# anacarsi/ss25_Hierarchical_Multiscale_Image_Classification

Measured on AMD Instinct MI355X. Metric: 224x224 patches/sec (ResNet18 fwd), higher is better.
Workload: dtype bf16; 1 GPU; resnet18_fwd_872k_patches_bf16; input=uint8 HWC patches resident in HBM, outputs=features[B,512] + logits[B,2] + labels, weights=seeded random init, parallelism=single GPU

## Files before the change

ss25_hierarchical_multiscale_image_classification_amd/csrc/block16_c64.h:

```cpp
#pragma once
#include "halo16.h"

namespace hipac {

typedef __attribute__((ext_vector_type(2))) short s16x2;
__device__ __forceinline__ unsigned relu_pk(unsigned v) {
  return __builtin_bit_cast(unsigned, __builtin_elementwise_max(__builtin_bit_cast(s16x2, v), s16x2{0, 0}));
}

constexpr int kBlkRing = 30;
constexpr int kBlkXPitch = 18 * 128;
constexpr int kBlkIPitch = 16 * 128;
constexpr int kBlkXBytes = 32 * kBlkXPitch + 512;
constexpr int kBlkIBytes = 32 * kBlkIPitch + 256;
constexpr int kBlkRsBytes = 2 * 6144 + 2 * 4096;

#ifndef HIPAC_BLK16_AHEAD
#define HIPAC_BLK16_AHEAD 1
#endif

template <typename T, int NP, int PITCH>
__device__ __forceinline__ void c64_strip16_mfma(const typename Elem<T>::frag (&wreg)[9][2][2], const int (&lb)[NP][3],
                                                 const float* __restrict__ bl, f32x4 (&acc)[2 * NP][2]) {
  using frag = typename Elem<T>::frag;
  constexpr int NR = 2 * NP;
#pragma unroll
  for (int t = 0; t < 2; ++t) {
    const f32x4 b = *reinterpret_cast<const f32x4*>(bl + 16 * t);
#pragma unroll
    for (int i = 0; i < NR; ++i) acc[i][t] = b;
  }
  asm volatile("s_waitcnt lgkmcnt(0)" ::: "memory");
  constexpr int AH = HIPAC_BLK16_AHEAD;
  frag fr[AH + 1][NR];
  auto rd = [&](auto S, auto I) {
    constexpr int s = decltype(S)::value, i = decltype(I)::value;
    constexpr int tap = s >> 1, kk = s & 1, kh = tap / 3, kw = tap % 3;
    lds_read16<((i & 1) + kh) * PITCH>(fr[s % (AH + 1)][i], (unsigned)(lb[i >> 1][kw] ^ (kk << 6)));
  };
  __builtin_amdgcn_s_setprio(1);
  static_for<AH>([&](auto S) { static_for<NR>([&](auto I) { rd(S, I); }); });
  static_for<18>([&](auto S) {
    constexpr int s = decltype(S)::value, tap = s >> 1, kk = s & 1;
    static_for<NR>([&](auto I) {
      constexpr int i = decltype(I)::value;
      if constexpr (s + AH < 18) rd(std::integral_constant<int, s + AH>{}, I);
      constexpr int full = (18 - 1 - s < AH - 1 ? 18 - 1 - s : AH - 1);
      wait_lgkmcnt<(NR - 1 - i) + full * NR + (s + AH < 18 ? i + 1 : 0)>();
      Asm16<T>::mfma(acc[i][0], wreg[tap][kk][0], fr[s % (AH + 1)][i]);
      Asm16<T>::mfma(acc[i][1], wreg[tap][kk][1], fr[s % (AH + 1)][i]);
    });
  });
  __builtin_amdgcn_s_setprio(0);
  asm volatile("s_nop 7\n\ts_nop 7\n\ts_nop 3" ::: "memory");
}

template <typename T>
__global__ __launch_bounds__(512, 2) void block16_c64_kernel(const T* __restrict__ in, const T* __restrict__ w1,
                                                             const float* __restrict__ b1, const T* __restrict__ w2,
                                                             const float* __restrict__ b2, T* __restrict__ out,
                                                             int n_img) {
  using E = Elem<T>;
  using frag = typename E::frag;
  using vec4 = typename E::vec4;
  constexpr int H = 56, W = 56, C = 64, RING = kBlkRing, XP = kBlkXPitch, IP = kBlkIPitch;
  __shared__ __attribute__((aligned(1024))) unsigned char smem[kBlkXBytes + kBlkIBytes + kBlkRsBytes + 512];
  unsigned char* const Xr = smem;
  unsigned char* const Ir = smem + kBlkXBytes;
  float* const Bl = reinterpret_cast<float*>(smem + kBlkXBytes + kBlkIBytes + kBlkRsBytes);

  const int tid = threadIdx.x, lane = tid & 63;
  const int wave = __builtin_amdgcn_readfirstlane(tid >> 6);
  const int team = wave >> 2, tw = wave & 3, nh = tw & 1, mh = tw >> 1;
  const int n16 = lane & 15, g = lane >> 4;
  const int lx = n16 < 4 ? 2 * n16 : (n16 < 12 ? 2 * n16 - 7 : 2 * n16 - 16);
  unsigned char* const Rw = smem + kBlkXBytes + kBlkIBytes + (mh == 0 ? nh * 6144 : 2 * 6144 + nh * 4096);

  if (tid < 64) Bl[tid] = b1[tid];
  else if (tid < 128) Bl[tid] = b2[tid - 64];

  const int xcd = blockIdx.x & 7, slot = blockIdx.x >> 3, nslots = gridDim.x >> 3;
  const int n_x = n_img > xcd ? (n_img - xcd + 7) >> 3 : 0;
  const int nst = 4 * n_x;
  const int ns = nst > slot ? (nst - slot + nslots - 1) / nslots : 0;
  if (ns == 0) return;

  frag wreg[9][2][2];
  {
    const char* wb = reinterpret_cast<const char*>(team ? w2 : w1) + (size_t)(nh * 32 + n16) * (9 * C * 2) + 16 * g;
#pragma unroll
    for (int tap = 0; tap < 9; ++tap)
#pragma unroll
      for (int kk = 0; kk < 2; ++kk)
#pragma unroll
        for (int t = 0; t < 2; ++t) wreg[tap][kk][t] = *reinterpret_cast<const frag*>(wb + t * 16 * (9 * C * 2) + tap * 128 + kk * 64);
  }

  const rsrc_t x_rsrc = make_rsrc(in, n_img * (H * W * C * 2));

  constexpr int NKP = 5;
  int relo[NKP];
#pragma unroll
  for (int kp = 0; kp < NKP; ++kp) {
    const int q = 8 * (tw + 4 * kp) + (lane >> 3);
    const int rr = (q * 3641) >> 16;
    const int j = q - 18 * rr;
    const int c = (lane & 7) ^ ((j >> 1) & 7);
    relo[kp] = (((rr * W + j) << 7) + (c << 4)) | (j < 2 ? 1 : 0) | (j >= 16 ? 2 : 0) | (rr == 0 ? 4 : 0) | (rr >= 1 ? 8 : 0);
  }
  auto x_rows = [&](int img, int x0, int L0, int rb, int np, int rowmask) {
    const int sb = ((img * H + L0 - 1) * W + x0 - 2) << 7;
    const int smask = (x0 == 0 ? 1 : 0) | (x0 == 42 ? 2 : 0) | rowmask;
    static_for<NKP>([&](auto KP) {
      constexpr int kp = decltype(KP)::value;
      const int p = tw + 4 * kp;
      if (p < np) {
        asm volatile("" : "+v"(relo[kp]));
        const int off = (relo[kp] & smask) ? (int)0x80000000 : (relo[kp] & ~15) + sb;
        buffer_load_lds16(x_rsrc, Xr + rb * XP + p * 1024, off, 0);
      }
    });
  };
  auto x_group = [&](int img, int x0, int gq) {
    const int rb = 8 * gq >= RING ? 8 * gq - RING : 8 * gq;
    x_rows(img, x0, 8 * gq, rb, gq == 7 ? 5 : 18, gq == 0 ? 4 : (gq == 7 ? 8 : 0));
    if (gq == 3) x_rows(img, x0, RING, 0, 5, 0);
  };
  auto strip_img = [&](int k) { return (((slot + k * nslots) >> 2) << 3) + xcd; };
  auto strip_x0 = [&](int k) { return ((slot + k * nslots) & 3) * 14; };

  const int lds_base = (int)(unsigned)(size_t)(__attribute__((address_space(3))) unsigned char*)smem;
  int la[3];
#pragma unroll
  for (int kw = 0; kw < 3; ++kw) {
    const int j = lx + kw;
    la[kw] = (j << 7) + (((((j >> 1) & 7)) ^ g) << 4) + (team ? kBlkXBytes : 0) + lds_base;
  }
  const int iw_lane = (lx << 7) + ((g & 1) << 3);
  const int iw_pos = ((nh << 2) + (g >> 1)) ^ ((lx >> 1) & 7);
  const float* const bl = Bl + team * 64 + nh * 32 + 4 * g;

#pragma unroll
  for (int tap = 0; tap < 9; ++tap)
#pragma unroll
    for (int kk = 0; kk < 2; ++kk)
#pragma unroll
      for (int t = 0; t < 2; ++t) asm volatile("" ::"v"(wreg[tap][kk][t]));
  if (team == 0) {
    x_group(strip_img(0), strip_x0(0), 0);
    x_group(strip_img(0), strip_x0(0), 1);
    wait_vmcnt<0>();
  }
  asm volatile("s_waitcnt lgkmcnt(0)" ::: "memory");
  __builtin_amdgcn_s_barrier();

  const int n_steps = 7 * ns;
  f32x4 acc[4][2];
  int pend_n = 0, pend_y = 0;
  const int rs_px = lane >> 2;
  const int rs_off = (((rs_px < 14 ? rs_px : 13)) * C + nh * 32 + 8 * ((lane & 3) ^ ((rs_px >> 2) & 3))) * 2;
  auto fetch_resid = [&](int pix0, int y0, int sl) {
    const int sb = (pix0 + y0 * W) << 7;
#pragma unroll
    for (int rho = 0; rho < 2; ++rho) buffer_load_lds16(x_rsrc, Rw + sl * 2048 + rho * 1024, rs_off + rho * (W * C * 2), sb);
  };
  const int rs_rd = lx * 64 + 8 * (g & 1);
  const int rs_sw = (lx >> 2) & 3;
  const int out_lane = (lx * C + nh * 32 + 16 * (g & 1) + 8 * (g >> 1)) * 2;
  auto epilogue_b = [&](auto A0, int pix0, int y0, int sl) {
    constexpr int a0 = decltype(A0)::value;
#pragma unroll
    for (int rho = 0; rho < 2; ++rho) {
      unsigned P[2][2];
#pragma unroll
      for (int t = 0; t < 2; ++t) {
        const vec4 rv = *reinterpret_cast<const vec4*>(Rw + sl * 2048 + rho * 1024 + rs_rd + (((2 * t + (g >> 1)) ^ rs_sw) << 4));
        const f32x4& a = acc[a0 + rho][t];
        P[t][0] = relu_pk(PackPair<T>::pack_rn(a[0] + (float)rv[0], a[1] + (float)rv[1]));
        P[t][1] = relu_pk(PackPair<T>::pack_rn(a[2] + (float)rv[2], a[3] + (float)rv[3]));
      }
      permlane16_swap(P[0][0], P[1][0]);
      permlane16_swap(P[0][1], P[1][1]);
      char* const dst = reinterpret_cast<char*>(out) + ((size_t)(unsigned)(pix0 + (y0 + rho) * W) << 7) + out_lane;
      if (lx < 14) store16_out(dst, u32x4{P[0][0], P[0][1], P[1][0], P[1][1]});
    }
  };
  int pend_pix = 0, pend_sl = 0;
  auto flush_b = [&]() {
    if (pend_n) {
      wait_vmcnt<0>();
      epilogue_b(std::integral_constant<int, 0>{}, pend_pix, pend_y, pend_sl);
      if (pend_n == 2) epilogue_b(std::integral_constant<int, 2>{}, pend_pix, pend_y + 2, pend_sl + 1);
      pend_n = 0;
    }
  };
  auto step_barrier = [&]() {
    asm volatile("s_waitcnt lgkmcnt(0)" ::: "memory");
    __builtin_amdgcn_s_barrier();
  };
  if (team == 0) {
    for (int G = 0; G <= n_steps; ++G) {
      if (G < n_steps) {
        const int k = G / 7, m = G - 7 * k;
        const int img = strip_img(k), x0 = strip_x0(k);
        if (m <= 4) x_group(img, x0, m + 2);
        else if (m == 5) {
          x_group(img, x0, 7);
          if (k + 1 < ns) x_group(strip_img(k + 1), strip_x0(k + 1), 0);
        } else if (k + 1 < ns) x_group(strip_img(k + 1), strip_x0(k + 1), 1);
        if (m == 0 || m == 6)
          *reinterpret_cast<u32x2*>(Ir + (m == 0 ? 0 : 27) * IP + tw * 512 + lane * 8) = u32x2{0u, 0u};
        const int y0a = 8 * m + 4 * mh;
        int lb[2][3];
#pragma unroll
        for (int p = 0; p < 2; ++p) {
          const int y0 = y0a + 2 * p;
          const int wbase = (y0 >= RING ? y0 - RING : y0) * XP;
#pragma unroll
          for (int kw = 0; kw < 3; ++kw) lb[p][kw] = la[kw] + wbase;
        }
        c64_strip16_mfma<T, 2, XP>(wreg, lb, bl, acc);
        const bool col_ok = !((x0 == 0 && lx == 0) || (x0 == 42 && lx == 15));
#pragma unroll
        for (int i = 0; i < 4; ++i) {
          const int Lr = y0a + i + 1;
          const bool twice = Lr == RING || Lr == RING + 1;
          unsigned char* const dst = Ir + (Lr >= RING ? Lr - RING : Lr) * IP + iw_lane;
          unsigned char* const dst2 = Ir + Lr * IP + iw_lane;
#pragma unroll
          for (int t = 0; t < 2; ++t) {
            u32x2 pk;
            pk[0] = relu_pk(PackPair<T>::pack_rn(acc[i][t][0], acc[i][t][1]));
            pk[1] = relu_pk(PackPair<T>::pack_rn(acc[i][t][2], acc[i][t][3]));
            if (!col_ok) pk = u32x2{0u, 0u};
            *reinterpret_cast<u32x2*>(dst + ((iw_pos ^ (2 * t)) << 4)) = pk;
            if (twice) *reinterpret_cast<u32x2*>(dst2 + ((iw_pos ^ (2 * t)) << 4)) = pk;
          }
        }
      }
      wait_vmcnt<0>();
      step_barrier();
    }
  } else {
    for (int G = 0; G <= n_steps; ++G) {
      flush_b();
      if (G >= 1) {
        const int k = (G - 1) / 7, mp = G - 7 * k;
        int yp = 8 * mp - 10 + 4 * mh, ys = -1;
        bool has_pair = true;
        if (mp == 1) {
          if (mh == 0) yp = 0;
          else has_pair = false, ys = 4;
        } else if (mp == 7) {
          if (mh == 0) yp = 46, ys = 50;
          else yp = 52;
        }
        const int pix0 = strip_img(k) * (H * W) + strip_x0(k);
        if (has_pair) {
          fetch_resid(pix0, yp, 0);
          fetch_resid(pix0, yp + 2, 1);
        }
        if (ys >= 0) fetch_resid(pix0, ys, has_pair ? 2 : 0);
        pend_pix = pix0;
        if (has_pair) {
          int lb[2][3];
#pragma unroll
          for (int p = 0; p < 2; ++p) {
            const int y0 = yp + 2 * p;
            const int wbase = (y0 >= RING ? y0 - RING : y0) * IP;
#pragma unroll
            for (int kw = 0; kw < 3; ++kw) lb[p][kw] = la[kw] + wbase;
          }
          c64_strip16_mfma<T, 2, IP>(wreg, lb, bl, acc);
          pend_n = 2, pend_y = yp, pend_sl = 0;
        }
        if (ys >= 0) {
          flush_b();
          int lb[1][3];
          const int wbase = (ys >= RING ? ys - RING : ys) * IP;
#pragma unroll
          for (int kw = 0; kw < 3; ++kw) lb[0][kw] = la[kw] + wbase;
          f32x4(&acc1)[2][2] = reinterpret_cast<f32x4(&)[2][2]>(acc[0]);
          c64_strip16_mfma<T, 1, IP>(wreg, lb, bl, acc1);
          pend_n = 1, pend_y = ys, pend_sl = has_pair ? 2 : 0;
        }
      }
      step_barrier();
    }
    flush_b();
  }
}

}
```

ss25_hierarchical_multiscale_image_classification_amd/csrc/conv_bf16.hip:

```cpp
#include "trunk.h"
namespace hipac {
int run_trunk_bf16(const Net& net, const Plan& p, char* ws, const void* xin, int n_early, int img_off, int n_late,
                   hipStream_t s, int first, int last) {
  return run_trunk<__bf16>(net, p, ws, xin, n_early, img_off, n_late, s, first, last);
}
}

#ifdef HIPAC_HALO_STAMPS
extern "C" int hipac_debug_halo_stamps(unsigned long long* out8, int reset) {
  if (hipMemcpyFromSymbol(out8, HIP_SYMBOL(hipac::g_halo_stamps), 64) != hipSuccess) return 1;
  if (reset) {
    unsigned long long z[8] = {0};
    if (hipMemcpyToSymbol(HIP_SYMBOL(hipac::g_halo_stamps), z, 64) != hipSuccess) return 1;
  }
  return 0;
}
#endif
```

Measured before the change: 309,200 patches/s.

## Read residual shortcut from X ring in LDS instead of reloading from HBM

The second conv team now takes the residual input from the already-resident X ring buffer in LDS rather than issuing separate buffer loads into a dedicated residual staging area. To keep the needed rows alive long enough, the X ring grows to 32 rows plus 2 wrap rows, indexed per strip with a 58-row stride, and the load scheduling is rewritten around spans. This removes the redundant global reads, the residual LDS region and the vmcnt waits in the epilogue. In exchange it adds more complex ring indexing, a slightly larger X buffer, and extra LDS reads in team B.

Measured after the change: 311,100 patches/s (median of 6 runs). No clear change (+0.6%).

```diff
diff --git a/ss25_hierarchical_multiscale_image_classification_amd/csrc/block16_c64.h b/ss25_hierarchical_multiscale_image_classification_amd/csrc/block16_c64.h
--- a/ss25_hierarchical_multiscale_image_classification_amd/csrc/block16_c64.h
+++ b/ss25_hierarchical_multiscale_image_classification_amd/csrc/block16_c64.h
@@ -1,4 +1,5 @@
 #pragma once
+#include "block16_ring.h"
 #include "halo16.h"
 
 namespace hipac {
@@ -9,11 +10,8 @@
 }
 
 constexpr int kBlkRing = 30;
-constexpr int kBlkXPitch = 18 * 128;
 constexpr int kBlkIPitch = 16 * 128;
-constexpr int kBlkXBytes = 32 * kBlkXPitch + 512;
 constexpr int kBlkIBytes = 32 * kBlkIPitch + 256;
-constexpr int kBlkRsBytes = 2 * 6144 + 2 * 4096;
 
 #ifndef HIPAC_BLK16_AHEAD
 #define HIPAC_BLK16_AHEAD 1
@@ -64,17 +62,16 @@
   using frag = typename E::frag;
   using vec4 = typename E::vec4;
   constexpr int H = 56, W = 56, C = 64, RING = kBlkRing, XP = kBlkXPitch, IP = kBlkIPitch;
-  __shared__ __attribute__((aligned(1024))) unsigned char smem[kBlkXBytes + kBlkIBytes + kBlkRsBytes + 512];
+  __shared__ __attribute__((aligned(1024))) unsigned char smem[kBlkXBytes + kBlkIBytes + 512];
   unsigned char* const Xr = smem;
   unsigned char* const Ir = smem + kBlkXBytes;
-  float* const Bl = reinterpret_cast<float*>(smem + kBlkXBytes + kBlkIBytes + kBlkRsBytes);
+  float* const Bl = reinterpret_cast<float*>(smem + kBlkXBytes + kBlkIBytes);
 
   const int tid = threadIdx.x, lane = tid & 63;
   const int wave = __builtin_amdgcn_readfirstlane(tid >> 6);
   const int team = wave >> 2, tw = wave & 3, nh = tw & 1, mh = tw >> 1;
   const int n16 = lane & 15, g = lane >> 4;
   const int lx = n16 < 4 ? 2 * n16 : (n16 < 12 ? 2 * n16 - 7 : 2 * n16 - 16);
-  unsigned char* const Rw = smem + kBlkXBytes + kBlkIBytes + (mh == 0 ? nh * 6144 : 2 * 6144 + nh * 4096);
 
   if (tid < 64) Bl[tid] = b1[tid];
   else if (tid < 128) Bl[tid] = b2[tid - 64];
@@ -106,28 +103,36 @@
     const int rr = (q * 3641) >> 16;
     const int j = q - 18 * rr;
     const int c = (lane & 7) ^ ((j >> 1) & 7);
-    relo[kp] = (((rr * W + j) << 7) + (c << 4)) | (j < 2 ? 1 : 0) | (j >= 16 ? 2 : 0) | (rr == 0 ? 4 : 0) | (rr >= 1 ? 8 : 0);
-  }
-  auto x_rows = [&](int img, int x0, int L0, int rb, int np, int rowmask) {
+    relo[kp] = (((rr * W + j) << 7) + (c << 4)) | (j < 2 ? 1 : 0) | (j >= 16 ? 2 : 0) | (rr == 0 ? 4 : 0);
+  }
+  auto x_rows = [&](int img, int x0, int L0, int rb, int np) {
     const int sb = ((img * H + L0 - 1) * W + x0 - 2) << 7;
-    const int smask = (x0 == 0 ? 1 : 0) | (x0 == 42 ? 2 : 0) | rowmask;
+    const int smask = (x0 == 0 ? 1 : 0) | (x0 == 42 ? 2 : 0) | (L0 == 0 ? 4 : 0);
+    const int below = (H + 1 - L0) * (W * 128);
     static_for<NKP>([&](auto KP) {
       constexpr int kp = decltype(KP)::value;
       const int p = tw + 4 * kp;
       if (p < np) {
         asm volatile("" : "+v"(relo[kp]));
-        const int off = (relo[kp] & smask) ? (int)0x80000000 : (relo[kp] & ~15) + sb;
+        const int off = ((relo[kp] & smask) || relo[kp] >= below) ? (int)0x80000000 : (relo[kp] & ~15) + sb;
         buffer_load_lds16(x_rsrc, Xr + rb * XP + p * 1024, off, 0);
       }
     });
-  };
-  auto x_group = [&](int img, int x0, int gq) {
-    const int rb = 8 * gq >= RING ? 8 * gq - RING : 8 * gq;
-    x_rows(img, x0, 8 * gq, rb, gq == 7 ? 5 : 18, gq == 0 ? 4 : (gq == 7 ? 8 : 0));
-    if (gq == 3) x_rows(img, x0, RING, 0, 5, 0);
   };
   auto strip_img = [&](int k) { return (((slot + k * nslots) >> 2) << 3) + xcd; };
   auto strip_x0 = [&](int k) { return ((slot + k * nslots) & 3) * 14; };
+  auto x_request = [&](int k, int L0, int nrows) {
+    const int img = strip_img(k), x0 = strip_x0(k);
+#pragma unroll
+    for (int i = 0; i < 3; ++i) {
+      const Blk16Span sp = blk16_x_span(k, L0, nrows, i);
+      if (sp.nrows) x_rows(img, x0, sp.L0, sp.row, blk16_x_pieces(sp.nrows));
+    }
+  };
+  auto x_strip_head = [&](int k) {
+    x_request(k, 0, 2);
+    x_request(k, 2, 8);
+  };
 
   const int lds_base = (int)(unsigned)(size_t)(__attribute__((address_space(3))) unsigned char*)smem;
   int la[3];
@@ -147,8 +152,7 @@
 #pragma unroll
       for (int t = 0; t < 2; ++t) asm volatile("" ::"v"(wreg[tap][kk][t]));
   if (team == 0) {
-    x_group(strip_img(0), strip_x0(0), 0);
-    x_group(strip_img(0), strip_x0(0), 1);
+    x_strip_head(0);
     wait_vmcnt<0>();
   }
   asm volatile("s_waitcnt lgkmcnt(0)" ::: "memory");
@@ -157,27 +161,35 @@
   const int n_steps = 7 * ns;
   f32x4 acc[4][2];
   int pend_n = 0, pend_y = 0;
-  const int rs_px = lane >> 2;
-  const int rs_off = (((rs_px < 14 ? rs_px : 13)) * C + nh * 32 + 8 * ((lane & 3) ^ ((rs_px >> 2) & 3))) * 2;
-  auto fetch_resid = [&](int pix0, int y0, int sl) {
-    const int sb = (pix0 + y0 * W) << 7;
-#pragma unroll
-    for (int rho = 0; rho < 2; ++rho) buffer_load_lds16(x_rsrc, Rw + sl * 2048 + rho * 1024, rs_off + rho * (W * C * 2), sb);
-  };
-  const int rs_rd = lx * 64 + 8 * (g & 1);
-  const int rs_sw = (lx >> 2) & 3;
+  const int sc_j = lx + 2;
+  const int sc_lane = (sc_j << 7) + ((g & 1) << 3);
+  const int sc_pos = ((nh << 2) + (g >> 1)) ^ ((sc_j >> 1) & 7);
   const int out_lane = (lx * C + nh * 32 + 16 * (g & 1) + 8 * (g >> 1)) * 2;
-  auto epilogue_b = [&](auto A0, int pix0, int y0, int sl) {
+  auto add_shortcut = [&](auto NR_, int k, int y0) {
+    constexpr int NR = decltype(NR_)::value;
+    vec4 rv[NR][2];
+#pragma unroll
+    for (int i = 0; i < NR; ++i)
+#pragma unroll
+      for (int t = 0; t < 2; ++t)
+        rv[i][t] = *reinterpret_cast<const vec4*>(Xr + blk16_x_row(k, y0 + i + 1) * XP + sc_lane + ((sc_pos ^ (2 * t)) << 4));
+#pragma unroll
+    for (int i = 0; i < NR; ++i)
+#pragma unroll
+      for (int t = 0; t < 2; ++t)
+#pragma unroll
+        for (int e = 0; e < 4; ++e) acc[i][t][e] = acc[i][t][e] + (float)rv[i][t][e];
+  };
+  auto epilogue_b = [&](auto A0, int pix0, int y0) {
     constexpr int a0 = decltype(A0)::value;
 #pragma unroll
     for (int rho = 0; rho < 2; ++rho) {
       unsigned P[2][2];
 #pragma unroll
       for (int t = 0; t < 2; ++t) {
-        const vec4 rv = *reinterpret_cast<const vec4*>(Rw + sl * 2048 + rho * 1024 + rs_rd + (((2 * t + (g >> 1)) ^ rs_sw) << 4));
         const f32x4& a = acc[a0 + rho][t];
-        P[t][0] = relu_pk(PackPair<T>::pack_rn(a[0] + (float)rv[0], a[1] + (float)rv[1]));
-        P[t][1] = relu_pk(PackPair<T>::pack_rn(a[2] + (float)rv[2], a[3] + (float)rv[3]));
+        P[t][0] = relu_pk(PackPair<T>::pack_rn(a[0], a[1]));
+        P[t][1] = relu_pk(PackPair<T>::pack_rn(a[2], a[3]));
       }
       permlane16_swap(P[0][0], P[1][0]);
       permlane16_swap(P[0][1], P[1][1]);
@@ -185,12 +197,11 @@
       if (lx < 14) store16_out(dst, u32x4{P[0][0], P[0][1], P[1][0], P[1][1]});
     }
   };
-  int pend_pix = 0, pend_sl = 0;
+  int pend_pix = 0;
   auto flush_b = [&]() {
     if (pend_n) {
-      wait_vmcnt<0>();
-      epilogue_b(std::integral_constant<int, 0>{}, pend_pix, pend_y, pend_sl);
-      if (pend_n == 2) epilogue_b(std::integral_constant<int, 2>{}, pend_pix, pend_y + 2, pend_sl + 1);
+      epilogue_b(std::integral_constant<int, 0>{}, pend_pix, pend_y);
+      if (pend_n == 2) epilogue_b(std::integral_constant<int, 2>{}, pend_pix, pend_y + 2);
       pend_n = 0;
     }
   };
@@ -202,20 +213,16 @@
     for (int G = 0; G <= n_steps; ++G) {
       if (G < n_steps) {
         const int k = G / 7, m = G - 7 * k;
-        const int img = strip_img(k), x0 = strip_x0(k);
-        if (m <= 4) x_group(img, x0, m + 2);
-        else if (m == 5) {
-          x_group(img, x0, 7);
-          if (k + 1 < ns) x_group(strip_img(k + 1), strip_x0(k + 1), 0);
-        } else if (k + 1 < ns) x_group(strip_img(k + 1), strip_x0(k + 1), 1);
+        const int x0 = strip_x0(k);
+        if (m <= 5) x_request(k, 8 * m + 10, 8);
+        else if (k + 1 < ns) x_strip_head(k + 1);
         if (m == 0 || m == 6)
           *reinterpret_cast<u32x2*>(Ir + (m == 0 ? 0 : 27) * IP + tw * 512 + lane * 8) = u32x2{0u, 0u};
         const int y0a = 8 * m + 4 * mh;
         int lb[2][3];
 #pragma unroll
         for (int p = 0; p < 2; ++p) {
-          const int y0 = y0a + 2 * p;
-          const int wbase = (y0 >= RING ? y0 - RING : y0) * XP;
+          const int wbase = blk16_x_row(k, y0a + 2 * p) * XP;
 #pragma unroll
           for (int kw = 0; kw < 3; ++kw) lb[p][kw] = la[kw] + wbase;
         }
@@ -246,22 +253,10 @@
       flush_b();
       if (G >= 1) {
         const int k = (G - 1) / 7, mp = G - 7 * k;
-        int yp = 8 * mp - 10 + 4 * mh, ys = -1;
-        bool has_pair = true;
-        if (mp == 1) {
-          if (mh == 0) yp = 0;
-          else has_pair = false, ys = 4;
-        } else if (mp == 7) {
-          if (mh == 0) yp = 46, ys = 50;
-          else yp = 52;
-        }
-        const int pix0 = strip_img(k) * (H * W) + strip_x0(k);
-        if (has_pair) {
-          fetch_resid(pix0, yp, 0);
-          fetch_resid(pix0, yp + 2, 1);
-        }
-        if (ys >= 0) fetch_resid(pix0, ys, has_pair ? 2 : 0);
-        pend_pix = pix0;
+        const Blk16BRows br = blk16_b_rows(mp, mh);
+        const int yp = br.yp, ys = br.ys;
+        const bool has_pair = br.has_pair;
+        pend_pix = strip_img(k) * (H * W) + strip_x0(k);
         if (has_pair) {
           int lb[2][3];
 #pragma unroll
@@ -272,7 +267,8 @@
             for (int kw = 0; kw < 3; ++kw) lb[p][kw] = la[kw] + wbase;
           }
           c64_strip16_mfma<T, 2, IP>(wreg, lb, bl, acc);
-          pend_n = 2, pend_y = yp, pend_sl = 0;
+          add_shortcut(std::integral_constant<int, 4>{}, k, yp);
+          pend_n = 2, pend_y = yp;
         }
         if (ys >= 0) {
           flush_b();
@@ -282,7 +278,8 @@
           for (int kw = 0; kw < 3; ++kw) lb[0][kw] = la[kw] + wbase;
           f32x4(&acc1)[2][2] = reinterpret_cast<f32x4(&)[2][2]>(acc[0]);
           c64_strip16_mfma<T, 1, IP>(wreg, lb, bl, acc1);
-          pend_n = 1, pend_y = ys, pend_sl = has_pair ? 2 : 0;
+          add_shortcut(std::integral_constant<int, 2>{}, k, ys);
+          pend_n = 1, pend_y = ys;
         }
       }
       step_barrier();
diff --git a/ss25_hierarchical_multiscale_image_classification_amd/csrc/block16_ring.h b/ss25_hierarchical_multiscale_image_classification_amd/csrc/block16_ring.h
--- /dev/null
+++ b/ss25_hierarchical_multiscale_image_classification_amd/csrc/block16_ring.h
@@ -0,0 +1,42 @@
+#pragma once
+
+namespace hipac {
+
+constexpr int kBlkXPitch = 18 * 128;
+constexpr int kBlkXRing = 32;
+constexpr int kBlkXRows = kBlkXRing + 2;
+constexpr int kBlkXBytes = kBlkXRows * kBlkXPitch + 512;
+constexpr int kBlkStripRows = 58;
+
+constexpr int blk16_x_row(int strip, int L) { return (kBlkStripRows * strip + L) & (kBlkXRing - 1); }
+constexpr int blk16_x_pieces(int nrows) { return (nrows * 18 + 7) >> 3; }
+
+struct Blk16Span {
+  int L0, row, nrows;
+};
+constexpr Blk16Span blk16_x_span(int strip, int L0, int nrows, int i) {
+  const int r0 = blk16_x_row(strip, L0);
+  const int n1 = nrows < kBlkXRing - r0 ? nrows : kBlkXRing - r0;
+  if (i == 0) return Blk16Span{L0, r0, n1};
+  if (i == 1) return Blk16Span{L0 + n1, 0, nrows - n1};
+  if (r0 == 0) return Blk16Span{L0, kBlkXRing, 2};
+  return Blk16Span{L0 + n1, kBlkXRing, n1 < nrows ? 2 : 0};
+}
+
+struct Blk16BRows {
+  int yp, ys;
+  bool has_pair;
+};
+constexpr Blk16BRows blk16_b_rows(int mp, int mh) {
+  Blk16BRows r{8 * mp - 10 + 4 * mh, -1, true};
+  if (mp == 1) {
+    if (mh == 0) r.yp = 0;
+    else r.has_pair = false, r.ys = 4;
+  } else if (mp == 7) {
+    if (mh == 0) r.yp = 46, r.ys = 50;
+    else r.yp = 52;
+  }
+  return r;
+}
+
+}
```

## Deepen LDS prefetch pipeline in block16 conv MFMA loop and prioritize flush

Applied to the files above, without the earlier changes.

Replaces the per-tap fragment prefetch (one step ahead) with a flat ring of 8 fragment registers and a configurable prefetch distance of 6 reads, so LDS loads run further ahead of the MFMAs. Bias is now loaded with LDS reads into the last accumulator and copied into the others, so its wait folds into the first fragment wait instead of a full lgkmcnt(0) drain. The residual epilogue hoists all LDS residual reads before the math and raises wave priority during the flush. Optional timestamp instrumentation is added behind a debug macro. The deeper ring raises VGPR pressure, which could hurt occupancy under the 512x2 launch bounds.

Result: no change. 311,200 patches/s before, 314,100 patches/s after, median of 6 (+0.9%).

```diff
diff --git a/ss25_hierarchical_multiscale_image_classification_amd/csrc/block16_c64.h b/ss25_hierarchical_multiscale_image_classification_amd/csrc/block16_c64.h
--- a/ss25_hierarchical_multiscale_image_classification_amd/csrc/block16_c64.h
+++ b/ss25_hierarchical_multiscale_image_classification_amd/csrc/block16_c64.h
@@ -14,42 +14,57 @@
 constexpr int kBlkXBytes = 32 * kBlkXPitch + 512;
 constexpr int kBlkIBytes = 32 * kBlkIPitch + 256;
 constexpr int kBlkRsBytes = 2 * 6144 + 2 * 4096;
-
-#ifndef HIPAC_BLK16_AHEAD
-#define HIPAC_BLK16_AHEAD 1
-#endif
-
-template <typename T, int NP, int PITCH>
+constexpr int kBlkStampPairs = 12;
+#ifdef HIPAC_HALO_STAMPS
+static __device__ unsigned long long g_blk16_stamps[20];
+#endif
+
+#ifndef HIPAC_BLK16_DIST
+#define HIPAC_BLK16_DIST 6
+#endif
+#ifndef HIPAC_BLK16_PRIO_FLUSH
+#define HIPAC_BLK16_PRIO_FLUSH 3
+#endif
+
+template <typename T, int NP, int PITCH, typename Mark>
 __device__ __forceinline__ void c64_strip16_mfma(const typename Elem<T>::frag (&wreg)[9][2][2], const int (&lb)[NP][3],
-                                                 const float* __restrict__ bl, f32x4 (&acc)[2 * NP][2]) {
+                                                 unsigned bl, f32x4 (&acc)[2 * NP][2], Mark&& mark) {
   using frag = typename Elem<T>::frag;
   constexpr int NR = 2 * NP;
-#pragma unroll
-  for (int t = 0; t < 2; ++t) {
-    const f32x4 b = *reinterpret_cast<const f32x4*>(bl + 16 * t);
-#pragma unroll
-    for (int i = 0; i < NR; ++i) acc[i][t] = b;
-  }
-  asm volatile("s_waitcnt lgkmcnt(0)" ::: "memory");
-  constexpr int AH = HIPAC_BLK16_AHEAD;
-  frag fr[AH + 1][NR];
-  auto rd = [&](auto S, auto I) {
-    constexpr int s = decltype(S)::value, i = decltype(I)::value;
+  constexpr int NF = 18 * NR;
+  constexpr int R = 8, D = HIPAC_BLK16_DIST;
+  static_assert(D >= 1 && D <= R - 2, "a slot is rewritten two MFMA pairs after its reader at the earliest");
+  static_assert(D + 2 < 16, "lgkmcnt range");
+  frag fr[R];
+  auto rd = [&](auto F) {
+    constexpr int f = decltype(F)::value, s = f / NR, i = f % NR;
     constexpr int tap = s >> 1, kk = s & 1, kh = tap / 3, kw = tap % 3;
-    lds_read16<((i & 1) + kh) * PITCH>(fr[s % (AH + 1)][i], (unsigned)(lb[i >> 1][kw] ^ (kk << 6)));
-  };
+    lds_read16<((i & 1) + kh) * PITCH>(fr[f % R], (unsigned)(lb[i >> 1][kw] ^ (kk << 6)));
+  };
+  asm volatile("" ::: "memory");
   __builtin_amdgcn_s_setprio(1);
-  static_for<AH>([&](auto S) { static_for<NR>([&](auto I) { rd(S, I); }); });
-  static_for<18>([&](auto S) {
-    constexpr int s = decltype(S)::value, tap = s >> 1, kk = s & 1;
-    static_for<NR>([&](auto I) {
-      constexpr int i = decltype(I)::value;
-      if constexpr (s + AH < 18) rd(std::integral_constant<int, s + AH>{}, I);
-      constexpr int full = (18 - 1 - s < AH - 1 ? 18 - 1 - s : AH - 1);
-      wait_lgkmcnt<(NR - 1 - i) + full * NR + (s + AH < 18 ? i + 1 : 0)>();
-      Asm16<T>::mfma(acc[i][0], wreg[tap][kk][0], fr[s % (AH + 1)][i]);
-      Asm16<T>::mfma(acc[i][1], wreg[tap][kk][1], fr[s % (AH + 1)][i]);
-    });
+  lds_read16<0>(acc[NR - 1][0], bl);
+  lds_read16<64>(acc[NR - 1][1], bl);
+  static_for<(D < NF ? D : NF)>([&](auto F) { rd(F); });
+  static_for<NF>([&](auto F) {
+    constexpr int f = decltype(F)::value, s = f / NR, i = f % NR, tap = s >> 1, kk = s & 1;
+    if constexpr (f == kBlkStampPairs) mark(std::integral_constant<int, 1>{});
+    if constexpr (f == NF - kBlkStampPairs) mark(std::integral_constant<int, 2>{});
+    if constexpr (f + D < NF) rd(std::integral_constant<int, f + D>{});
+    constexpr int behind = NF - 1 - f < D ? NF - 1 - f : D;
+    if constexpr (f == 0) {
+      asm volatile("s_waitcnt lgkmcnt(%2)" : "+v"(acc[NR - 1][0]), "+v"(acc[NR - 1][1]) : "n"(behind));
+      mark(std::integral_constant<int, 0>{});
+    } else {
+      wait_lgkmcnt<behind>();
+    }
+    if constexpr (f < NR - 1) {
+      if constexpr (f > 0) asm volatile("" : "+v"(acc[NR - 1][0]), "+v"(acc[NR - 1][1]));
+      acc[i][0] = acc[NR - 1][0];
+      acc[i][1] = acc[NR - 1][1];
+    }
+    Asm16<T>::mfma(acc[i][0], wreg[tap][kk][0], fr[f % R]);
+    Asm16<T>::mfma(acc[i][1], wreg[tap][kk][1], fr[f % R]);
   });
   __builtin_amdgcn_s_setprio(0);
   asm volatile("s_nop 7\n\ts_nop 7\n\ts_nop 3" ::: "memory");
@@ -138,7 +153,7 @@
   }
   const int iw_lane = (lx << 7) + ((g & 1) << 3);
   const int iw_pos = ((nh << 2) + (g >> 1)) ^ ((lx >> 1) & 7);
-  const float* const bl = Bl + team * 64 + nh * 32 + 4 * g;
+  const unsigned bl = (unsigned)(lds_base + kBlkXBytes + kBlkIBytes + kBlkRsBytes + (team * 64 + nh * 32 + 4 * g) * 4);
 
 #pragma unroll
   for (int tap = 0; tap < 9; ++tap)
@@ -155,6 +170,19 @@
   __builtin_amdgcn_s_barrier();
 
   const int n_steps = 7 * ns;
+#ifdef HIPAC_HALO_STAMPS
+  unsigned long long z_sum[11] = {0, 0, 0, 0, 0, 0, 0, 0, 0, 0, 0}, z_tf = 0, z_th = 0, z_tt = 0, z_tv = 0, z_tr = 0;
+  auto mark = [&](auto K) {
+    HALO_STAMP(z_now);
+    if constexpr (decltype(K)::value == 2) z_tt = z_now;
+    else if constexpr (decltype(K)::value == 1) z_th = z_th ? z_th : z_now;
+    else z_tf = z_tf ? z_tf : z_now;
+  };
+  HALO_STAMP(z_t0v);
+  unsigned long long z_t0 = z_t0v;
+#else
+  auto mark = [](auto) {};
+#endif
   f32x4 acc[4][2];
   int pend_n = 0, pend_y = 0;
   const int rs_px = lane >> 2;
@@ -167,14 +195,21 @@
   const int rs_rd = lx * 64 + 8 * (g & 1);
   const int rs_sw = (lx >> 2) & 3;
   const int out_lane = (lx * C + nh * 32 + 16 * (g & 1) + 8 * (g >> 1)) * 2;
-  auto epilogue_b = [&](auto A0, int pix0, int y0, int sl) {
+  auto resid_rows = [&](vec4 (&rv)[2][2], int sl) {
+#pragma unroll
+    for (int rho = 0; rho < 2; ++rho)
+#pragma unroll
+      for (int t = 0; t < 2; ++t)
+        rv[rho][t] = *reinterpret_cast<const vec4*>(Rw + sl * 2048 + rho * 1024 + rs_rd + (((2 * t + (g >> 1)) ^ rs_sw) << 4));
+  };
+  auto epilogue_b = [&](auto A0, int pix0, int y0, const vec4 (&rvs)[2][2]) {
     constexpr int a0 = decltype(A0)::value;
 #pragma unroll
     for (int rho = 0; rho < 2; ++rho) {
       unsigned P[2][2];
 #pragma unroll
       for (int t = 0; t < 2; ++t) {
-        const vec4 rv = *reinterpret_cast<const vec4*>(Rw + sl * 2048 + rho * 1024 + rs_rd + (((2 * t + (g >> 1)) ^ rs_sw) << 4));
+        const vec4 rv = rvs[rho][t];
         const f32x4& a = acc[a0 + rho][t];
         P[t][0] = relu_pk(PackPair<T>::pack_rn(a[0] + (float)rv[0], a[1] + (float)rv[1]));
         P[t][1] = relu_pk(PackPair<T>::pack_rn(a[2] + (float)rv[2], a[3] + (float)rv[3]));
@@ -189,8 +224,22 @@
   auto flush_b = [&]() {
     if (pend_n) {
       wait_vmcnt<0>();
-      epilogue_b(std::integral_constant<int, 0>{}, pend_pix, pend_y, pend_sl);
-      if (pend_n == 2) epilogue_b(std::integral_constant<int, 2>{}, pend_pix, pend_y + 2, pend_sl + 1);
+      __builtin_amdgcn_s_setprio(HIPAC_BLK16_PRIO_FLUSH);
+#ifdef HIPAC_HALO_STAMPS
+      HALO_STAMP(z_v);
+      z_tv = z_v;
+#endif
+      vec4 rv[2][2][2];
+      resid_rows(rv[0], pend_sl);
+      if (pend_n == 2) resid_rows(rv[1], pend_sl + 1);
+#ifdef HIPAC_HALO_STAMPS
+      asm volatile("" ::: "memory");
+      HALO_STAMP(z_r);
+      z_tr = z_r;
+#endif
+      epilogue_b(std::integral_constant<int, 0>{}, pend_pix, pend_y, rv[0]);
+      if (pend_n == 2) epilogue_b(std::integral_constant<int, 2>{}, pend_pix, pend_y + 2, rv[1]);
+      __builtin_amdgcn_s_setprio(0);
       pend_n = 0;
     }
   };
@@ -219,7 +268,8 @@
 #pragma unroll
           for (int kw = 0; kw < 3; ++kw) lb[p][kw] = la[kw] + wbase;
         }
-        c64_strip16_mfma<T, 2, XP>(wreg, lb, bl, acc);
+        c64_strip16_mfma<T, 2, XP>(wreg, lb, bl, acc, mark);
+        HALO_STAMP(z_ts);
         const bool col_ok = !((x0 == 0 && lx == 0) || (x0 == 42 && lx == 15));
 #pragma unroll
         for (int i = 0; i < 4; ++i) {
@@ -237,13 +287,40 @@
             if (twice) *reinterpret_cast<u32x2*>(dst2 + ((iw_pos ^ (2 * t)) << 4)) = pk;
           }
         }
+#ifdef HIPAC_HALO_STAMPS
+        HALO_STAMP(z_te);
+        wait_vmcnt<0>();
+        HALO_STAMP(z_tw);
+        z_sum[0] += z_tf - z_t0, z_sum[1] += z_ts - z_tf, z_sum[2] += z_te - z_ts, z_sum[3] += z_tw - z_te;
+        z_sum[5] += 1, z_sum[6] += z_th - z_tf, z_sum[7] += z_ts - z_tt;
+        z_tf = z_th = 0;
+#endif
       }
       wait_vmcnt<0>();
+#ifdef HIPAC_HALO_STAMPS
+      HALO_STAMP(z_ta);
       step_barrier();
-    }
+      HALO_STAMP(z_tb);
+      if (G < n_steps) z_sum[4] += z_tb - z_ta;
+      z_t0 = z_tb;
+#else
+      step_barrier();
+#endif
+    }
+#ifdef HIPAC_HALO_STAMPS
+    if (lane == 0)
+      for (int q = 0; q < 8; ++q) atomicAdd(&g_blk16_stamps[q], z_sum[q]);
+#endif
   } else {
     for (int G = 0; G <= n_steps; ++G) {
+#ifdef HIPAC_HALO_STAMPS
+      z_tv = z_tr = z_t0;
       flush_b();
+      HALO_STAMP(z_tfl);
+      const unsigned long long z_dv = z_tv - z_t0, z_dr = z_tr - z_t0;
+#else
+      flush_b();
+#endif
       if (G >= 1) {
         const int k = (G - 1) / 7, mp = G - 7 * k;
         int yp = 8 * mp - 10 + 4 * mh, ys = -1;
@@ -262,6 +339,7 @@
         }
         if (ys >= 0) fetch_resid(pix0, ys, has_pair ? 2 : 0);
         pend_pix = pix0;
+        HALO_STAMP(z_t1);
         if (has_pair) {
           int lb[2][3];
 #pragma unroll
@@ -271,7 +349,7 @@
 #pragma unroll
             for (int kw = 0; kw < 3; ++kw) lb[p][kw] = la[kw] + wbase;
           }
-          c64_strip16_mfma<T, 2, IP>(wreg, lb, bl, acc);
+          c64_strip16_mfma<T, 2, IP>(wreg, lb, bl, acc, mark);
           pend_n = 2, pend_y = yp, pend_sl = 0;
         }
         if (ys >= 0) {
@@ -281,13 +359,32 @@
 #pragma unroll
           for (int kw = 0; kw < 3; ++kw) lb[0][kw] = la[kw] + wbase;
           f32x4(&acc1)[2][2] = reinterpret_cast<f32x4(&)[2][2]>(acc[0]);
-          c64_strip16_mfma<T, 1, IP>(wreg, lb, bl, acc1);
+          c64_strip16_mfma<T, 1, IP>(wreg, lb, bl, acc1, mark);
           pend_n = 1, pend_y = ys, pend_sl = has_pair ? 2 : 0;
         }
+#ifdef HIPAC_HALO_STAMPS
+        HALO_STAMP(z_ts);
+        z_sum[0] += z_t1 - z_t0, z_sum[1] += z_tf - z_t0, z_sum[2] += z_ts - z_tf;
+        z_sum[4] += (has_pair ? 144 : 0) + (ys >= 0 ? 72 : 0), z_sum[5] += 1, z_sum[6] += z_th - z_tf, z_sum[7] += z_ts - z_tt;
+        z_sum[8] += z_dv, z_sum[9] += z_dr, z_sum[10] += z_tfl - z_t0;
+        z_tf = z_th = 0;
+#endif
       }
+#ifdef HIPAC_HALO_STAMPS
+      HALO_STAMP(z_ta);
       step_barrier();
+      HALO_STAMP(z_tb);
+      if (G >= 1) z_sum[3] += z_tb - z_ta;
+      z_t0 = z_tb;
+#else
+      step_barrier();
+#endif
     }
     flush_b();
+#ifdef HIPAC_HALO_STAMPS
+    if (lane == 0)
+      for (int q = 0; q < 11; ++q) atomicAdd(&g_blk16_stamps[8 + q], z_sum[q]);
+#endif
   }
 }
 
diff --git a/ss25_hierarchical_multiscale_image_classification_amd/csrc/conv_bf16.hip b/ss25_hierarchical_multiscale_image_classification_amd/csrc/conv_bf16.hip
--- a/ss25_hierarchical_multiscale_image_classification_amd/csrc/conv_bf16.hip
+++ b/ss25_hierarchical_multiscale_image_classification_amd/csrc/conv_bf16.hip
@@ -15,4 +15,12 @@
   }
   return 0;
 }
+extern "C" int hipac_debug_blk16_stamps(unsigned long long* out20, int reset) {
+  if (hipMemcpyFromSymbol(out20, HIP_SYMBOL(hipac::g_blk16_stamps), 160) != hipSuccess) return 1;
+  if (reset) {
+    unsigned long long z[20] = {0};
+    if (hipMemcpyToSymbol(HIP_SYMBOL(hipac::g_blk16_stamps), z, 160) != hipSuccess) return 1;
+  }
+  return 0;
+}
 #endif
```
